# maneymarkus/BERT4Rec

Measured on AMD Instinct MI355X. Metric: masked positions/sec, higher is better.
Workload: dtype f32 (split products on the 16-bit matrix cores, fp32 accumulate: bf16 hi/lo x3 in the encoder, fp16 hi/lo x3 logits + x2 value products in the masked-LM head; softmax / LayerNorm / AdamW in fp32)

## Files before the change

bert4rec_amd/build.py:

```python
from __future__ import annotations

import os
import subprocess
import sys

HERE = os.path.dirname(os.path.abspath(__file__))
CSRC = os.path.join(HERE, "csrc")
SOURCES = ["b4r_gemm.hip", "b4r_gemm_rx.hip", "b4r_rowops.hip", "b4r_attn.hip", "b4r_attn_rx.hip", "b4r_attn64.hip", "b4r_head32.hip", "b4r_ffn_rx.hip", "b4r_ffn32w.hip", "b4r_attn_block.hip", "b4r_attn32.hip", "b4r_rank.hip", "b4r_rank_full.hip", "b4r_embed_proj.hip", "b4r_model.hip"]
OUT = os.path.join(HERE, "libb4r_hip.so")


def _newer(target: str, deps) -> bool:
    if not os.path.exists(target):
        return False
    t = os.path.getmtime(target)
    return all(os.path.getmtime(d) <= t for d in deps)


def build_library(force: bool = False, verbose: bool = True) -> str:
    srcs = [os.path.join(CSRC, s) for s in SOURCES]
    headers = [os.path.join(CSRC, h) for h in sorted(os.listdir(CSRC)) if h.endswith(".h")]
    deps = srcs + headers + [os.path.join(os.path.dirname(HERE), "include", "b4r.h")]
    if not force and _newer(OUT, deps):
        return OUT
    hipcc = os.environ.get("HIPCC", "/opt/rocm/bin/hipcc")
    objs = []
    procs = []
    for s in srcs:
        o = os.path.splitext(s)[0] + ".o"
        objs.append(o)
        cmd = [hipcc, "--offload-arch=gfx950", "-O3", "-std=c++17", "-fPIC", "-c", s, "-o", o]
        if verbose:
            print(" ".join(cmd), flush=True)
        procs.append((cmd, subprocess.Popen(cmd)))
    for cmd, p in procs:
        if p.wait() != 0:
            raise RuntimeError("hipcc failed: " + " ".join(cmd))
    cmd = [hipcc, "--offload-arch=gfx950", "-shared", "-fPIC", "-o", OUT] + objs
    if verbose:
        print(" ".join(cmd), flush=True)
    subprocess.check_call(cmd)
    return OUT


if __name__ == "__main__":
    build_library(force="--force" in sys.argv)
```

bert4rec_amd/csrc/b4r_gemm_rx.hip:

```cpp
#include <stdlib.h>

#include "b4r_common.h"

typedef __bf16 bf16x8 __attribute__((ext_vector_type(8)));
typedef __bf16 bf16x4 __attribute__((ext_vector_type(4)));
typedef float f32x8 __attribute__((ext_vector_type(8)));
typedef short s16x4 __attribute__((ext_vector_type(4)));

namespace {

constexpr int ST_LD = 32;
constexpr int STAGE_FLOATS = 4 * 32 * ST_LD;
constexpr int BROW_MAX = 36;
constexpr size_t KN_LDS_BYTES = STAGE_FLOATS * sizeof(float);
constexpr size_t NK_LDS_BYTES = STAGE_FLOATS * sizeof(float) + 2 * 2 * 32 * BROW_MAX * 4;

struct RxP {
  const float* A; const float* B; float* C; const float* bias; float* C2; const float* R;
  int lda, ldb, ldc, ldc2, ldr;
  int M, N, K;
  int n_store;
  int n_splits, steps_per_split;
  int n_items;
  int k_chunks_per_split;
// ... 873 lines not shown
#pragma unroll
      for (int e = 0; e < 4; ++e) {
        va[e] = live ? va[e] : 0.f;
        vb[e] = live ? vb[e] : 0.f;
      }
      if (B_DROP) vb = b4r_drop4(dctx, vb, (uint64_t)row * (uint64_t)p.No + (uint64_t)cb);
      cs += vb;
      csa += va;
      const int off = tn_img_off(lrow, c4);
      bf16x4 ah, al, bh, bl;
      b4r_split4(va, ah, al);
      b4r_split4(vb, bh, bl);
      *reinterpret_cast<bf16x4*>(s_tn + off) = ah;
      if constexpr (TERMS == 3) *reinterpret_cast<bf16x4*>(s_tn + PLANE + off) = al;
      *reinterpret_cast<bf16x4*>(s_tn + 2 * PLANE + off) = bh;
      if constexpr (TERMS == 3) *reinterpret_cast<bf16x4*>(s_tn + 3 * PLANE + off) = bl;
    }
  };
  const int qq = (lane & 15) >> 2, pp = lane & 3, gb = (lane >> 4) & 1;
  const int tr_a = tn_img_off(8 * h + qq, 4 * (2 * wm + gb) + pp);
  const int tr_b = tn_img_off(8 * h + qq, 4 * (2 * wn + gb) + pp);
  typedef __attribute__((address_space(3))) s16x4* lds_ptr;
  auto tr8 = [&](int plane, int addr, int kb) {
    const char* src = s_tn + plane * PLANE + addr + kb * (16 * 128);
    const s16x4 lo4 = __builtin_amdgcn_ds_read_tr16_b64_v4i16((lds_ptr)(src));
    const s16x4 hi4 = __builtin_amdgcn_ds_read_tr16_b64_v4i16((lds_ptr)(src + 4 * 128));
    return __builtin_bit_cast(bf16x8, __builtin_shufflevector(lo4, hi4, 0, 1, 2, 3, 4, 5, 6, 7));
  };

  f32x16 acc;
#pragma unroll
  for (int i = 0; i < 16; ++i) acc[i] = 0.f;
  bf16x8 wh[KS / 16], wl[KS / 16];
  if (DGRAD) {
#pragma unroll
    for (int kb = 0; kb < KS / 16; ++kb)
      split8(load8_contig(p.W + (int64_t)(i0 + 32 * wn + r) * p.ldw + 16 * kb + 8 * h), wh[kb], wl[kb]);
  }
  auto dgrad = [&](int k0) {
    f32x16 dx, gp;
#pragma unroll
    for (int i = 0; i < 16; ++i) dx[i] = 0.f;
    if (DGRAD >= 2) {
#pragma unroll
      for (int reg = 0; reg < 16; ++reg) {
        const int row = min(k0 + 32 * wm + (reg & 3) + 8 * (reg >> 2) + 4 * h, p.R - 1);
        gp[reg] = p.G[(int64_t)row * p.ldg + i0 + 32 * wn + r];
      }
    }
#pragma unroll
    for (int kb = 0; kb < KS / 16; ++kb) {
      const char* src = s_tn + 2 * PLANE + tn_img_off(32 * wm + r, 4 * kb + 2 * h);
      dx = mfma3<TERMS>(*reinterpret_cast<const bf16x8*>(src), *reinterpret_cast<const bf16x8*>(src + PLANE), wh[kb], wl[kb], dx);
    }
#pragma unroll
    for (int reg = 0; reg < 16; ++reg) {
      const int row = k0 + 32 * wm + (reg & 3) + 8 * (reg >> 2) + 4 * h;
      float v = dx[reg];
      if (DGRAD == 2) v *= b4r_gelu_grad_fast(gp[reg]);
      if (DGRAD == 3) v *= b4r_act_grad<true>(p.act, gp[reg]);
      if (row < r_end) p.dX[(int64_t)row * p.lddx + i0 + 32 * wn + r] = v;
    }
  };
  auto products = [&]() {
#pragma unroll
    for (int kb = 0; kb < KS / 16; ++kb)
      acc = mfma3<TERMS>(tr8(0, tr_a, kb), tr8(1, tr_a, kb), tr8(2, tr_b, kb), tr8(3, tr_b, kb), acc);
  };
  Chunk c0, c1;
  if (r_begin < r_end) fetch(c0, r_begin);
  for (int k0 = r_begin; k0 < r_end; k0 += 2 * KS) {
    fetch(c1, k0 + KS);
    __syncthreads();
    stash(c0, k0);
    __syncthreads();
    products();
    if (DGRAD) dgrad(k0);
    if (k0 + KS >= r_end) break;
    fetch(c0, k0 + 2 * KS);
    __syncthreads();
    stash(c1, k0 + KS);
    __syncthreads();
    products();
    if (DGRAD) dgrad(k0 + KS);
  }

  if (do_cs || do_csa) {
    __syncthreads();
    float* red = reinterpret_cast<float*>(s_tn);
    *reinterpret_cast<f32x4*>(red + srow * 64 + 4 * c4) = cs;
    *reinterpret_cast<f32x4*>(red + 1024 + srow * 64 + 4 * c4) = csa;
    __syncthreads();
    if (tid < 128) {
      const int which = tid >> 6, c = tid & 63;
      float sum = 0.f;
#pragma unroll
      for (int g = 0; g < 16; ++g) sum += red[which * 1024 + g * 64 + c];
      if (which == 0 && do_cs && j0 + c < p.No) p.colsum_slab[(int64_t)z * p.No + j0 + c] = sum;
      if (which == 1 && do_csa && i0 + c < p.Mo) p.colsum_a_slab[(int64_t)z * p.Mo + i0 + c] = sum;
    }
  }
  float* slab = p.slab + (int64_t)z * p.Mo * p.No;
  const int col = j0 + 32 * wn + r;
#pragma unroll
  for (int reg = 0; reg < 16; ++reg) {
    const int row = i0 + 32 * wm + (reg & 3) + 8 * (reg >> 2) + 4 * h;
    if (row < p.Mo && col < p.No) slab[(int64_t)row * p.No + col] = acc[reg];
  }
}

template <int KS, bool B_DROP, int DGRAD, int TERMS = 3>
__global__ __launch_bounds__(256) void rx_gemm_tn_kernel(RxTnP p) {
  rx_gemm_tn_body<KS, B_DROP, DGRAD, TERMS>(p, (int)blockIdx.x);
}
#ifndef TN_PAIR_OCC
#define TN_PAIR_OCC 3
#endif
template <int KS, bool B_DROP0, bool B_DROP1, int TERMS = 3>
__global__ __launch_bounds__(256, TN_PAIR_OCC) void rx_gemm_tn_pair_kernel(RxTnP p0, RxTnP p1, int n0) {
  if ((int)blockIdx.x < n0) rx_gemm_tn_body<KS, B_DROP0, 0, TERMS>(p0, (int)blockIdx.x);
  else rx_gemm_tn_body<KS, B_DROP1, 0, TERMS>(p1, (int)blockIdx.x - n0);
}

constexpr int TN128_KS = 32;
__device__ __forceinline__ int tn128_off(int row, int c4) {
  return row * 256 + 32 * ((c4 >> 2) ^ (2 * (row & 3))) + 8 * (c4 & 3);
}
template <bool B_DROP, int TERMS = 3>
__global__ __launch_bounds__(512, 2) void rx_gemm_tn128_kernel(RxTnP p) {
  constexpr int KS = TN128_KS, NLD = KS / 16, PLANE = KS * 256;
  extern __shared__ __attribute__((aligned(16))) char s_tn[];
  const int tid = threadIdx.x, lane = tid & 63, wave = __builtin_amdgcn_readfirstlane(tid >> 6);
  const int r = lane & 31, h = lane >> 5;
  const int wm = wave >> 2, wn = wave & 3;
  const int n_items = p.tiles_i * p.tiles_j * p.S;
  const int item = xcd_logical_id((int)blockIdx.x, n_items);
  if (item >= n_items) return;
  const int z = item / (p.tiles_i * p.tiles_j);
  const int t = item % (p.tiles_i * p.tiles_j);
  const int ti = t / p.tiles_j, tj = t % p.tiles_j;
  const int i0 = ti * 128, j0 = tj * 128;
  const int r_begin = min(p.R, z * p.chunk), r_end = min(p.R, r_begin + p.chunk);
  const bool do_cs = p.colsum_slab != nullptr && ti == 0;
  const bool do_csa = p.colsum_a_slab != nullptr && tj == 0;
  const DropCtx dctx = b4r_drop_ctx(p.drop);

  const int c4 = tid & 31, srow = tid >> 5;
  const int ca = i0 + 4 * c4, cb = j0 + 4 * c4;
  struct Chunk { f32x4 a[NLD], b[NLD]; };
  auto fetch = [&](Chunk& c, int k0) {
#pragma unroll
    for (int j = 0; j < NLD; ++j) {
      const int row = min(k0 + srow + 16 * j, p.R - 1);
      c.a[j] = *reinterpret_cast<const f32x4*>(p.A + (int64_t)row * p.lda + ca);
      c.b[j] = *reinterpret_cast<const f32x4*>(p.B + (int64_t)row * p.ldb + cb);
    }
  };
  f32x4 cs = {0.f, 0.f, 0.f, 0.f}, csa = {0.f, 0.f, 0.f, 0.f};
  auto stash = [&](const Chunk& c, int k0) {
#pragma unroll
    for (int j = 0; j < NLD; ++j) {
      const int lrow = srow + 16 * j, row = k0 + lrow;
      const bool live = row < r_end;
      f32x4 va = c.a[j], vb = c.b[j];
#pragma unroll
      for (int e = 0; e < 4; ++e) {
        va[e] = live ? va[e] : 0.f;
        vb[e] = live ? vb[e] : 0.f;
      }
      if (B_DROP) vb = b4r_drop4(dctx, vb, (uint64_t)row * (uint64_t)p.No + (uint64_t)cb);
      cs += vb;
      csa += va;
      const int off = tn128_off(lrow, c4);
      bf16x4 ah, al, bh, bl;
      b4r_split4(va, ah, al);
      b4r_split4(vb, bh, bl);
      *reinterpret_cast<bf16x4*>(s_tn + off) = ah;
      if constexpr (TERMS == 3) *reinterpret_cast<bf16x4*>(s_tn + PLANE + off) = al;
      *reinterpret_cast<bf16x4*>(s_tn + 2 * PLANE + off) = bh;
      if constexpr (TERMS == 3) *reinterpret_cast<bf16x4*>(s_tn + 3 * PLANE + off) = bl;
    }
  };
  const int qq = (lane & 15) >> 2, pp = lane & 3, gb = (lane >> 4) & 1;
  int tr_a[2];
#pragma unroll
  for (int b = 0; b < 2; ++b) tr_a[b] = tn128_off(8 * h + qq, 4 * (2 * (2 * wm + b) + gb) + pp);
  const int tr_b = tn128_off(8 * h + qq, 4 * (2 * wn + gb) + pp);
  typedef __attribute__((address_space(3))) s16x4* lds_ptr;
  auto tr8 = [&](int plane, int addr, int kb) {
    const char* src = s_tn + plane * PLANE + addr + kb * (16 * 256);
    const s16x4 lo4 = __builtin_amdgcn_ds_read_tr16_b64_v4i16((lds_ptr)(src));
    const s16x4 hi4 = __builtin_amdgcn_ds_read_tr16_b64_v4i16((lds_ptr)(src + 4 * 256));
    return __builtin_bit_cast(bf16x8, __builtin_shufflevector(lo4, hi4, 0, 1, 2, 3, 4, 5, 6, 7));
  };
  f32x16 acc[2];
#pragma unroll
  for (int bi = 0; bi < 2; ++bi)
#pragma unroll
    for (int i = 0; i < 16; ++i) acc[bi][i] = 0.f;
  auto products = [&]() {
#pragma unroll
    for (int kb = 0; kb < KS / 16; ++kb) {
      const bf16x8 bh = tr8(2, tr_b, kb), bl = tr8(3, tr_b, kb);
#pragma unroll
      for (int bi = 0; bi < 2; ++bi) acc[bi] = mfma3<TERMS>(tr8(0, tr_a[bi], kb), tr8(1, tr_a[bi], kb), bh, bl, acc[bi]);
    }
  };
  Chunk c0, c1;
  if (r_begin < r_end) fetch(c0, r_begin);
  for (int k0 = r_begin; k0 < r_end; k0 += 2 * KS) {
    fetch(c1, k0 + KS);
    __syncthreads();
    stash(c0, k0);
    __syncthreads();
    products();
    if (k0 + KS >= r_end) break;
    fetch(c0, k0 + 2 * KS);
    __syncthreads();
    stash(c1, k0 + KS);
    __syncthreads();
    products();
  }
  if (do_cs || do_csa) {
    __syncthreads();
    float* red = reinterpret_cast<float*>(s_tn);
    *reinterpret_cast<f32x4*>(red + srow * 128 + 4 * c4) = cs;
    *reinterpret_cast<f32x4*>(red + 2048 + srow * 128 + 4 * c4) = csa;
    __syncthreads();
    if (tid < 256) {
      const int which = tid >> 7, c = tid & 127;
      float sum = 0.f;
#pragma unroll
      for (int g = 0; g < 16; ++g) sum += red[which * 2048 + g * 128 + c];
      if (which == 0 && do_cs) p.colsum_slab[(int64_t)z * p.No + j0 + c] = sum;
      if (which == 1 && do_csa) p.colsum_a_slab[(int64_t)z * p.Mo + i0 + c] = sum;
    }
  }
  float* slab = p.slab + (int64_t)z * p.Mo * p.No;
  const int col = j0 + 32 * wn + r;
#pragma unroll
  for (int bi = 0; bi < 2; ++bi)
#pragma unroll
    for (int reg = 0; reg < 16; ++reg) {
      const int row = i0 + 32 * (2 * wm + bi) + (reg & 3) + 8 * (reg >> 2) + 4 * h;
      slab[(int64_t)row * p.No + col] = acc[bi][reg];
    }
}

inline bool tn_wide_tiles(int Mo, int No) {
  return Mo >= 128 && No >= 128 && Mo % 128 == 0 && No % 128 == 0;
}

constexpr int TN_KS = 64;

constexpr int TN_CAP1 = 512;
constexpr int TN_TARGET = 512;
constexpr int TN_TARGET_WIDE = 256;
int rx_tn_split(int R, int Mo, int No) {
  const bool wide = tn_wide_tiles(Mo, No);
  const int tw = wide ? 128 : 64;
  const int tiles = b4r_cdiv(Mo, tw) * b4r_cdiv(No, tw);
  int S = b4r_cdiv(wide ? TN_TARGET_WIDE : TN_TARGET, tiles);
  const int max_s = b4r_cdiv(R, 2 * TN_KS);
  if (S > max_s) S = max_s;
  const int cap = tiles == 1 ? TN_CAP1 : 256;
  if (S > cap) S = cap;
  if (S < 1) S = 1;
  return S;
}

inline bool vec_ok(const void* ptr, int ld) { return ptr != nullptr && b4r_aligned16(ptr) && (ld % 4 == 0); }
inline int up4i(int x) { return (x + 3) & ~3; }

}

bool b4r_gemm_rx_supported(const b4r_gemm_desc* d) {
  const bool k_small = (d->K == 64 || d->K == 32);
  const bool k_loop = (d->K > 64 && d->K % 64 == 0);
  if (!(k_small || k_loop) || d->M % 32 != 0 || d->N < 4) return false;
  if (!vec_ok(d->A, d->lda) || !vec_ok(d->C, d->ldc)) return false;
  if (d->b_is_nk && !vec_ok(d->B, d->ldb)) return false;
  const int ns = up4i(d->N);
  if (ns != d->N && (!d->c_pad_scratch || ns > d->ldc)) return false;
  const int epi = d->epilogue;
  if (epi_has_r(epi) && (!vec_ok(d->R, d->ldr) || ns > d->ldr)) return false;
  if (epi == B4R_EPI_BIAS_GELU && (!vec_ok(d->C2, d->ldc2) || ns > d->ldc2)) return false;
  if (epi == B4R_EPI_BIAS_DROP_RES_LN || epi == B4R_EPI_BIAS_GELU_LN) {
    if (d->N != 64 || d->K < 64 || d->K % WIDE_KC != 0 || d->b_is_nk || d->a_dropout) return false;
    if (!vec_ok(d->C2, d->ldc2) || d->ldc2 < 64 || !vec_ok(d->ln_gamma, 4) || !vec_ok(d->ln_beta, 4)) return false;
    if (epi == B4R_EPI_BIAS_GELU_LN && (!vec_ok(d->C3, d->ldc3) || d->ldc3 < 64)) return false;
  }
  if (epi == B4R_EPI_ADD_RES_LN_BWD) {
    if (d->N != 64 || d->K < 64 || d->K % WIDE_KC != 0 || !d->b_is_nk || d->a_dropout) return false;
    if (!vec_ok(d->C2, 4) || !vec_ok(d->ln_gamma, 4) || !d->ln_mean || !d->ln_rstd) return false;
    if (d->ln_ids) {
      if (!vec_ok(d->ln_table, 4) || !vec_ok(d->ln_pos, 4) || d->ln_L < 1 || d->ln_V < 1) return false;
    } else if (!vec_ok(d->ln_z, d->ln_ldz) || d->ln_ldz < 64) {
      return false;
    }
  }
  return true;
}

int b4r_gemm_rx_launch(const b4r_gemm_desc* d, hipStream_t stream) {
  RxP p;
  p.A = d->A; p.B = d->B; p.C = d->C; p.bias = d->bias; p.C2 = d->C2; p.R = d->R;
  p.lda = d->lda; p.ldb = d->ldb; p.ldc = d->ldc; p.ldc2 = d->ldc2; p.ldr = d->ldr;
  p.M = d->M; p.N = d->N; p.K = d->K;
  p.n_store = up4i(d->N);
  p.qscale = d->qscale; p.qcols = d->qcols;
  p.ln_gamma = d->ln_gamma; p.ln_beta = d->ln_beta; p.ln_mean = d->ln_mean; p.ln_rstd = d->ln_rstd; p.ln_eps = d->ln_eps;
  p.ln_z = d->ln_z; p.ln_ldz = d->ln_ldz;
  p.ln_ids = d->ln_ids; p.ln_table = d->ln_table; p.ln_pos = d->ln_pos; p.ln_L = d->ln_L; p.ln_V = d->ln_V;
  p.C3 = d->C3; p.ldc3 = d->ldc3;
  p.a_idx = d->a_gather_idx; p.a_add_per = d->a_gather_add_per; p.a_per = d->a_gather_per > 0 ? d->a_gather_per : 1;
  p.a_copy = d->a_copy; p.a_copy_ld = d->a_copy_ld;
  p.act = d->activation;
  p.drop = b4r_make_drop(d->rng, d->drop_stream, d->drop_rate, 1);
  p.k_chunks_per_split = d->K / 64 > 0 ? d->K / 64 : 1; p.slab_stride = 0;
  const bool a_drop = d->a_dropout && p.drop.rng != nullptr;
  const int mblocks = b4r_cdiv(d->M, 128);
  const int total_steps = b4r_cdiv(d->N, 32);
  constexpr int RX_TARGET = 1024;
  int splits = RX_TARGET / mblocks;
  if (splits > total_steps) splits = total_steps;
  if (splits < 1) splits = 1;
  p.steps_per_split = b4r_cdiv(total_steps, splits);
  p.n_splits = b4r_cdiv(total_steps, p.steps_per_split);
  p.n_items = mblocks * p.n_splits;
  dim3 grid(xcd_grid(p.n_items));
  if (p.n_splits > 4) p.n_items = -p.n_items;
  const bool one = b4r_gemm_terms() == 1;
  int rc = d->b_is_nk ? (one ? dispatch_rx<true, 1>(p, d->epilogue, a_drop, grid, stream)
                             : dispatch_rx<true, 3>(p, d->epilogue, a_drop, grid, stream))
                      : (one ? dispatch_rx<false, 1>(p, d->epilogue, a_drop, grid, stream)
                             : dispatch_rx<false, 3>(p, d->epilogue, a_drop, grid, stream));
  if (rc != B4R_OK) return rc;
  B4R_CHECK_LAUNCH(one ? "b4r_gemm_f32 (bf16)" : "b4r_gemm_f32 (bf16x3)");
  return B4R_OK;
}

bool b4r_gemm_rx_splitk_supported(const b4r_gemm_desc* d, int k_pad_ok) {
  const int Kp = (d->K + 63) & ~63;
  if (d->b_is_nk || d->epilogue != B4R_EPI_NONE || d->a_dropout) return false;
  if (Kp <= 64 || (Kp != d->K && (!k_pad_ok || d->lda < Kp))) return false;
  if (d->M % 32 != 0 || d->N % 4 != 0 || d->N > 128) return false;
  return vec_ok(d->A, d->lda) && d->B != nullptr;
}

int b4r_gemm_rx_splitk_launch(const b4r_gemm_desc* d, int splits, float* slabs, int* slabs_used, hipStream_t stream) {
  RxP p{};
  p.A = d->A; p.B = d->B; p.C = slabs; p.lda = d->lda; p.ldb = d->ldb; p.ldc = d->N;
  p.M = d->M; p.N = d->N; p.K = (d->K + 63) & ~63;
  p.n_store = d->N;
  p.qscale = 1.f;
  p.drop = b4r_make_drop(nullptr, 0, 0.f, 0);
  const int chunks = p.K / 64;
  p.k_chunks_per_split = b4r_cdiv(chunks, splits < 1 ? 1 : splits);
  p.slab_stride = (int64_t)d->M * d->N;
  *slabs_used = b4r_cdiv(chunks, p.k_chunks_per_split);
  if (b4r_gemm_terms() == 1) launch_kloop<false, B4R_EPI_NONE, false, 1>(p, stream);
  else launch_kloop<false, B4R_EPI_NONE, false, 3>(p, stream);
  B4R_CHECK_LAUNCH(b4r_gemm_terms() == 1 ? "gemm_splitk (bf16)" : "gemm_splitk (bf16x3)");
  return B4R_OK;
}

int b4r_launch_slab_reduce_full(const float* slab, int S, int Mo, int No, float* out, int ldo, int accumulate,
                                const float* cslab, float* colsum, const float* caslab, float* colsum_a, hipStream_t stream);

bool b4r_gemm_rx_tn_supported(const b4r_gemm_tn_desc* d) {
  if (!vec_ok(d->A, d->lda) || !vec_ok(d->B, d->ldb)) return false;
  return up4i(d->Mo) <= d->lda && up4i(d->No) <= d->ldb && d->Mo >= 4 && d->No >= 4;
}

int64_t b4r_gemm_rx_tn_scratch_floats(int R, int Mo, int No) {
  const int S = rx_tn_split(R, Mo, No);
  return (int64_t)S * Mo * No + (int64_t)S * No + (int64_t)S * Mo;
}

static RxTnP make_tn_params(const b4r_gemm_tn_desc* d, float* scratch, int S) {
  RxTnP p;
  p.A = d->A; p.B = d->B; p.lda = d->lda; p.ldb = d->ldb;
  p.R = d->R; p.Mo = d->Mo; p.No = d->No;
  const int tw = (tn_wide_tiles(d->Mo, d->No) && d->dgrad_out == nullptr) ? 128 : 64;
  p.tiles_i = b4r_cdiv(d->Mo, tw); p.tiles_j = b4r_cdiv(d->No, tw); p.S = S;
  p.chunk = b4r_cdiv(b4r_cdiv(d->R, S), TN_KS) * TN_KS;
  p.a_lim = up4i(d->Mo); p.b_lim = up4i(d->No);
  p.slab = scratch;
  p.colsum_slab = d->colsum ? scratch + (int64_t)S * d->Mo * d->No : nullptr;
  p.colsum_a_slab = d->colsum_a ? scratch + (int64_t)S * d->Mo * d->No + (int64_t)S * d->No : nullptr;
  p.drop = b4r_make_drop(d->rng, d->drop_stream, d->drop_rate, 1);
  p.W = d->dgrad_w; p.ldw = d->dgrad_ldw; p.dX = d->dgrad_out; p.lddx = d->dgrad_ldo; p.G = d->dgrad_gelu_pre; p.ldg = d->dgrad_ldg;
  p.act = d->activation;
  return p;
}

template <int TERMS>
static int rx_tn_launch(const b4r_gemm_tn_desc* d, float* scratch, hipStream_t stream) {
  const int S = rx_tn_split(d->R, d->Mo, d->No);
  const RxTnP p = make_tn_params(d, scratch, S);
  const bool b_drop = d->b_dropout && p.drop.rng != nullptr;
  const int dgrad = d->dgrad_out == nullptr ? 0 : !d->dgrad_gelu_pre ? 1 : d->activation != B4R_ACT_GELU ? 3 : 2;
  const int64_t items = (int64_t)p.tiles_i * p.tiles_j * S;
  dim3 grid(xcd_grid(items));
  if (dgrad == 0 && tn_wide_tiles(d->Mo, d->No)) {
    constexpr size_t lds128 = (size_t)4 * TN128_KS * 256;
    if (b_drop) hipLaunchKernelGGL((rx_gemm_tn128_kernel<true, TERMS>), grid, dim3(512), lds128, stream, p);
    else hipLaunchKernelGGL((rx_gemm_tn128_kernel<false, TERMS>), grid, dim3(512), lds128, stream, p);
    B4R_CHECK_LAUNCH(TERMS == 1 ? "b4r_gemm_tn_f32 (bf16, 128 x 128 tiles)" : "b4r_gemm_tn_f32 (bf16x3, 128 x 128 tiles)");
    return b4r_launch_slab_reduce_full(p.slab, S, d->Mo, d->No, d->out, d->ldo, d->accumulate, p.colsum_slab, d->colsum,
                                       p.colsum_a_slab, d->colsum_a, stream);
  }
  constexpr size_t lds = (size_t)4 * TN_KS * 128;
  static bool lds_raised = false;
  if (lds > 48 * 1024 && !lds_raised) {
    (void)hipFuncSetAttribute((const void*)rx_gemm_tn_kernel<TN_KS, true, 0, TERMS>, hipFuncAttributeMaxDynamicSharedMemorySize, (int)lds);
    (void)hipFuncSetAttribute((const void*)rx_gemm_tn_kernel<TN_KS, false, 0, TERMS>, hipFuncAttributeMaxDynamicSharedMemorySize, (int)lds);
    (void)hipFuncSetAttribute((const void*)rx_gemm_tn_kernel<TN_KS, true, 1, TERMS>, hipFuncAttributeMaxDynamicSharedMemorySize, (int)lds);
    (void)hipFuncSetAttribute((const void*)rx_gemm_tn_kernel<TN_KS, false, 1, TERMS>, hipFuncAttributeMaxDynamicSharedMemorySize, (int)lds);
    (void)hipFuncSetAttribute((const void*)rx_gemm_tn_kernel<TN_KS, true, 2, TERMS>, hipFuncAttributeMaxDynamicSharedMemorySize, (int)lds);
    (void)hipFuncSetAttribute((const void*)rx_gemm_tn_kernel<TN_KS, false, 2, TERMS>, hipFuncAttributeMaxDynamicSharedMemorySize, (int)lds);
    (void)hipFuncSetAttribute((const void*)rx_gemm_tn_kernel<TN_KS, true, 3, TERMS>, hipFuncAttributeMaxDynamicSharedMemorySize, (int)lds);
    (void)hipFuncSetAttribute((const void*)rx_gemm_tn_kernel<TN_KS, false, 3, TERMS>, hipFuncAttributeMaxDynamicSharedMemorySize, (int)lds);
    lds_raised = true;
  }
#define B4R_TN_LAUNCH(BD, DG) hipLaunchKernelGGL((rx_gemm_tn_kernel<TN_KS, BD, DG, TERMS>), grid, dim3(256), lds, stream, p)
  if (dgrad == 3) { if (b_drop) B4R_TN_LAUNCH(true, 3); else B4R_TN_LAUNCH(false, 3); }
  else if (dgrad == 2) { if (b_drop) B4R_TN_LAUNCH(true, 2); else B4R_TN_LAUNCH(false, 2); }
  else if (dgrad == 1) { if (b_drop) B4R_TN_LAUNCH(true, 1); else B4R_TN_LAUNCH(false, 1); }
  else if (b_drop) B4R_TN_LAUNCH(true, 0);
  else B4R_TN_LAUNCH(false, 0);
#undef B4R_TN_LAUNCH
  B4R_CHECK_LAUNCH(TERMS == 1 ? "b4r_gemm_tn_f32 (bf16)" : "b4r_gemm_tn_f32 (bf16x3)");
  return b4r_launch_slab_reduce_full(p.slab, S, d->Mo, d->No, d->out, d->ldo, d->accumulate, p.colsum_slab, d->colsum,
                                     p.colsum_a_slab, d->colsum_a, stream);
}

bool b4r_gemm_rx_tn_pair_supported(const b4r_gemm_tn_desc* d0, const b4r_gemm_tn_desc* d1) {
  if (tn_wide_tiles(d0->Mo, d0->No) || tn_wide_tiles(d1->Mo, d1->No)) return false;
  return b4r_gemm_rx_tn_supported(d0) && b4r_gemm_rx_tn_supported(d1) && !d0->dgrad_out && !d1->dgrad_out &&
         !(d1->b_dropout && d1->rng && d1->drop_rate > 0.f);
}
template <int TERMS>
static int rx_tn_pair_launch(const b4r_gemm_tn_desc* d0, float* scratch0, const b4r_gemm_tn_desc* d1, float* scratch1,
                             hipStream_t stream) {
  const int S0 = rx_tn_split(d0->R, d0->Mo, d0->No), S1 = rx_tn_split(d1->R, d1->Mo, d1->No);
  const RxTnP p0 = make_tn_params(d0, scratch0, S0), p1 = make_tn_params(d1, scratch1, S1);
  const bool drop0 = d0->b_dropout && p0.drop.rng != nullptr;
  const int n0 = (int)xcd_grid((int64_t)p0.tiles_i * p0.tiles_j * S0), n1 = (int)xcd_grid((int64_t)p1.tiles_i * p1.tiles_j * S1);
  constexpr size_t lds = (size_t)4 * TN_KS * 128;
  static bool lds_raised = false;
  if (lds > 48 * 1024 && !lds_raised) {
    (void)hipFuncSetAttribute((const void*)rx_gemm_tn_pair_kernel<TN_KS, true, false, TERMS>, hipFuncAttributeMaxDynamicSharedMemorySize, (int)lds);
    (void)hipFuncSetAttribute((const void*)rx_gemm_tn_pair_kernel<TN_KS, false, false, TERMS>, hipFuncAttributeMaxDynamicSharedMemorySize, (int)lds);
    lds_raised = true;
  }
  if (drop0) hipLaunchKernelGGL((rx_gemm_tn_pair_kernel<TN_KS, true, false, TERMS>), dim3(n0 + n1), dim3(256), lds, stream, p0, p1, n0);
  else hipLaunchKernelGGL((rx_gemm_tn_pair_kernel<TN_KS, false, false, TERMS>), dim3(n0 + n1), dim3(256), lds, stream, p0, p1, n0);
  B4R_CHECK_LAUNCH(TERMS == 1 ? "b4r_gemm_tn_f32 pair (bf16)" : "b4r_gemm_tn_f32 pair (bf16x3)");
  int rc = b4r_launch_slab_reduce_full(p0.slab, S0, d0->Mo, d0->No, d0->out, d0->ldo, d0->accumulate, p0.colsum_slab, d0->colsum,
                                       p0.colsum_a_slab, d0->colsum_a, stream);
  if (rc) return rc;
  return b4r_launch_slab_reduce_full(p1.slab, S1, d1->Mo, d1->No, d1->out, d1->ldo, d1->accumulate, p1.colsum_slab, d1->colsum,
                                     p1.colsum_a_slab, d1->colsum_a, stream);
}

int b4r_gemm_rx_tn_launch(const b4r_gemm_tn_desc* d, float* scratch, hipStream_t stream) {
  return b4r_gemm_terms() == 1 ? rx_tn_launch<1>(d, scratch, stream) : rx_tn_launch<3>(d, scratch, stream);
}
int b4r_gemm_rx_tn_pair_launch(const b4r_gemm_tn_desc* d0, float* scratch0, const b4r_gemm_tn_desc* d1, float* scratch1,
                               hipStream_t stream) {
  return b4r_gemm_terms() == 1 ? rx_tn_pair_launch<1>(d0, scratch0, d1, scratch1, stream)
                               : rx_tn_pair_launch<3>(d0, scratch0, d1, scratch1, stream);
}
```

Before: 18.89 million.

## Add dedicated fused gather-GEMM-GELU-LayerNorm kernel for MLM head transform

Routes the masked-LM head's dense transform (64x64 GEMM with bias, activation and LayerNorm epilogue, optional row gather) to a new specialized kernel. Each block stages the full 64x64 weight into LDS once, and each wave processes 16-row tiles in a grid-stride loop using bf16x3 split MFMA. Bias, GELU and LayerNorm are applied in registers, and pre-activation, activation, normalized output and mean/rstd are written directly. This replaces the generic wide-tile GEMM path for this shape to cut staging overhead and improve occupancy, at the cost of another kernel to maintain.

```diff
diff --git a/bert4rec_amd/build.py b/bert4rec_amd/build.py
--- a/bert4rec_amd/build.py
+++ b/bert4rec_amd/build.py
@@ -6,7 +6,7 @@
 
 HERE = os.path.dirname(os.path.abspath(__file__))
 CSRC = os.path.join(HERE, "csrc")
-SOURCES = ["b4r_gemm.hip", "b4r_gemm_rx.hip", "b4r_rowops.hip", "b4r_attn.hip", "b4r_attn_rx.hip", "b4r_attn64.hip", "b4r_head32.hip", "b4r_ffn_rx.hip", "b4r_ffn32w.hip", "b4r_attn_block.hip", "b4r_attn32.hip", "b4r_rank.hip", "b4r_rank_full.hip", "b4r_embed_proj.hip", "b4r_model.hip"]
+SOURCES = ["b4r_gemm.hip", "b4r_gemm_rx.hip", "b4r_rowops.hip", "b4r_attn.hip", "b4r_attn_rx.hip", "b4r_attn64.hip", "b4r_head32.hip", "b4r_ffn_rx.hip", "b4r_mlm_rx.hip", "b4r_ffn32w.hip", "b4r_attn_block.hip", "b4r_attn32.hip", "b4r_rank.hip", "b4r_rank_full.hip", "b4r_embed_proj.hip", "b4r_model.hip"]
 OUT = os.path.join(HERE, "libb4r_hip.so")
 
 
diff --git a/bert4rec_amd/csrc/b4r_gemm_rx.hip b/bert4rec_amd/csrc/b4r_gemm_rx.hip
--- a/bert4rec_amd/csrc/b4r_gemm_rx.hip
+++ b/bert4rec_amd/csrc/b4r_gemm_rx.hip
@@ -1199,7 +1199,15 @@
   return true;
 }
 
+bool b4r_mlm_rx_fwd_supported(const b4r_gemm_desc* d);
+void b4r_mlm_rx_fwd_launch(const b4r_gemm_desc* d, hipStream_t stream);
+
 int b4r_gemm_rx_launch(const b4r_gemm_desc* d, hipStream_t stream) {
+  if (b4r_gemm_terms() == 3 && b4r_mlm_rx_fwd_supported(d)) {
+    b4r_mlm_rx_fwd_launch(d, stream);
+    B4R_CHECK_LAUNCH("b4r_gemm_f32 (bf16x3)");
+    return B4R_OK;
+  }
   RxP p;
   p.A = d->A; p.B = d->B; p.C = d->C; p.bias = d->bias; p.C2 = d->C2; p.R = d->R;
   p.lda = d->lda; p.ldb = d->ldb; p.ldc = d->ldc; p.ldc2 = d->ldc2; p.ldr = d->ldr;
diff --git a/bert4rec_amd/csrc/b4r_mlm_rx.hip b/bert4rec_amd/csrc/b4r_mlm_rx.hip
--- /dev/null
+++ b/bert4rec_amd/csrc/b4r_mlm_rx.hip
@@ -0,0 +1,142 @@
+#include "b4r_block_tiles.h"
+
+namespace {
+
+constexpr int MW = 2;
+constexpr int WD_IMG = HID * HID * 4;
+constexpr int MLM_MAX_GRID = 2048;
+
+struct MlmFwdP {
+  const float* A; int lda;
+  const int64_t* idx; int64_t add_per; int per;
+  float* a_copy; int a_copy_ld;
+  const float* W; const float* bias; const float* gamma; const float* beta;
+  float* upre; int ld_upre; float* u; int ld_u; float* T; int ld_t; float* mean; float* rstd;
+  int M; float eps; int act;
+};
+
+__device__ __forceinline__ void mlm_fetch(const MlmFwdP& p, int t, int i, int g, f32x8 (&xv)[2]) {
+  const int m = min(16 * t + i, p.M - 1);
+  int64_t src = m;
+  if (p.idx) {
+    int64_t pos = p.idx[m];
+    pos = pos < 0 ? 0 : (pos >= p.add_per ? p.add_per - 1 : pos);
+    src = pos + (int64_t)(m / p.per) * p.add_per;
+  }
+#pragma unroll
+  for (int ks = 0; ks < 2; ++ks) xv[ks] = load8(p.A + src * p.lda + 32 * ks + 8 * g);
+}
+
+template <int ACT>
+__global__ __launch_bounds__(64 * MW) void mlm_fwd_kernel(MlmFwdP p) {
+  extern __shared__ __attribute__((aligned(16))) char smem_mlm[];
+  const int lane = threadIdx.x & 63, wave = __builtin_amdgcn_readfirstlane(threadIdx.x >> 6), i = lane & 15, g = lane >> 4;
+  const int ntiles = (p.M + 15) >> 4;
+  int t = blockIdx.x * MW + wave;
+  f32x8 xv[2];
+  if (t < ntiles) mlm_fetch(p, t, i, g, xv);
+  {
+    StageTurns s0, s1;
+    stage_request(s0, p.W, HID, HID, threadIdx.x, 64 * MW);
+    stage_request(s1, p.W, HID, HID, threadIdx.x + STAGE_U * 64 * MW, 64 * MW);
+    stage_commit(s0, smem_mlm, HID, HID, threadIdx.x, 64 * MW);
+    stage_commit(s1, smem_mlm, HID, HID, threadIdx.x + STAGE_U * 64 * MW, 64 * MW);
+  }
+  static_assert(2 * STAGE_U * 64 * MW * 4 == HID * HID, "two sets of turns cover Wd");
+  __syncthreads();
+
+  const LaneK lk = lane_consts(lane);
+  for (; t < ntiles; ) {
+    const int j = 16 * t + i;
+    const bool live = j < p.M;
+    if (p.a_copy && live) {
+#pragma unroll
+      for (int ks = 0; ks < 2; ++ks) {
+        float* dst = p.a_copy + (int64_t)j * p.a_copy_ld + 32 * ks + 8 * g;
+        *reinterpret_cast<f32x4*>(dst) = (f32x4){xv[ks][0], xv[ks][1], xv[ks][2], xv[ks][3]};
+        *reinterpret_cast<f32x4*>(dst + 4) = (f32x4){xv[ks][4], xv[ks][5], xv[ks][6], xv[ks][7]};
+      }
+    }
+    f32x4 acc[4];
+#pragma unroll
+    for (int hb = 0; hb < 4; ++hb) acc[hb] = (f32x4){0.f, 0.f, 0.f, 0.f};
+#pragma unroll
+    for (int ks = 0; ks < 2; ++ks) {
+      bf16x8 xh, xl;
+      split8(xv[ks], xh, xl);
+      const char* wt = smem_mlm + sub_base(2 * ks + lk.hi_tile, 0, 2);
+#pragma unroll
+      for (int hb = 0; hb < 4; ++hb) {
+        const char* th = wt + (hb >> 1) * 2 * SUB;
+        const int db = hb & 1;
+        acc[hb] = mfma3(tr_pair(th + lk.trk[db][0], th + lk.trk[db][1]), tr_pair(th + SUB + lk.trk[db][0], th + SUB + lk.trk[db][1]),
+                        xh, xl, acc[hb]);
+      }
+    }
+    f32x4 pre[4], z[4];
+    float s = 0.f;
+#pragma unroll
+    for (int hb = 0; hb < 4; ++hb) {
+      pre[hb] = acc[hb] + *reinterpret_cast<const f32x4*>(p.bias + 16 * hb + 4 * g);
+#pragma unroll
+      for (int e = 0; e < 4; ++e)
+        z[hb][e] = (ACT == B4R_ACT_GELU) ? b4r_gelu_fast(pre[hb][e]) : b4r_act_val<true>(b4r_act_id<ACT>(p.act), pre[hb][e]);
+      s += sum4(z[hb]);
+    }
+    const float mean = quad_sum(s) * (1.0f / HID);
+    float q = 0.f;
+#pragma unroll
+    for (int hb = 0; hb < 4; ++hb) {
+      const f32x4 d = z[hb] - mean;
+      q += sum4(d * d);
+    }
+    const float rstd = rsqrtf(quad_sum(q) * (1.0f / HID) + p.eps);
+    if (live) {
+#pragma unroll
+      for (int hb = 0; hb < 4; ++hb) {
+        const int c = 16 * hb + 4 * g;
+        const f32x4 gm = *reinterpret_cast<const f32x4*>(p.gamma + c);
+        const f32x4 be = *reinterpret_cast<const f32x4*>(p.beta + c);
+        f32x4 y;
+#pragma unroll
+        for (int e = 0; e < 4; ++e) {
+          const float inv = rstd * gm[e];
+          y[e] = z[hb][e] * inv + (be[e] - mean * inv);
+        }
+        *reinterpret_cast<f32x4*>(p.upre + (int64_t)j * p.ld_upre + c) = pre[hb];
+        *reinterpret_cast<f32x4*>(p.u + (int64_t)j * p.ld_u + c) = z[hb];
+        *reinterpret_cast<f32x4*>(p.T + (int64_t)j * p.ld_t + c) = y;
+      }
+      if (g == 0) {
+        if (p.mean) p.mean[j] = mean;
+        if (p.rstd) p.rstd[j] = rstd;
+      }
+    }
+    t += gridDim.x * MW;
+    if (t < ntiles) mlm_fetch(p, t, i, g, xv);
+  }
+}
+
+}
+
+bool b4r_mlm_rx_fwd_supported(const b4r_gemm_desc* d) {
+  return d->epilogue == B4R_EPI_BIAS_GELU_LN && d->N == HID && d->K == HID && !d->b_is_nk && !d->a_dropout && d->ldb == HID &&
+         b4r_aligned16(d->B) && b4r_aligned16(d->bias);
+}
+
+void b4r_mlm_rx_fwd_launch(const b4r_gemm_desc* d, hipStream_t stream) {
+  MlmFwdP p;
+  p.A = d->A; p.lda = d->lda;
+  p.idx = d->a_gather_idx; p.add_per = d->a_gather_add_per; p.per = d->a_gather_per > 0 ? d->a_gather_per : 1;
+  p.a_copy = d->a_copy; p.a_copy_ld = d->a_copy_ld;
+  p.W = d->B; p.bias = d->bias; p.gamma = d->ln_gamma; p.beta = d->ln_beta;
+  p.upre = d->C3; p.ld_upre = d->ldc3; p.u = d->C; p.ld_u = d->ldc; p.T = d->C2; p.ld_t = d->ldc2;
+  p.mean = d->ln_mean; p.rstd = d->ln_rstd;
+  p.M = d->M; p.eps = d->ln_eps; p.act = d->activation;
+  int grid = b4r_cdiv(b4r_cdiv(d->M, 16), MW);
+  if (grid > MLM_MAX_GRID) grid = MLM_MAX_GRID;
+  if (d->activation == B4R_ACT_GELU)
+    hipLaunchKernelGGL((mlm_fwd_kernel<B4R_ACT_GELU>), dim3(grid), dim3(64 * MW), WD_IMG, stream, p);
+  else
+    hipLaunchKernelGGL((mlm_fwd_kernel<B4R_ACT_ANY>), dim3(grid), dim3(64 * MW), WD_IMG, stream, p);
+}
```

Result: no change. 18.84 million (-0.2%).
